# kluonj/HelFEM

Measured on AMD Instinct MI355X. Metric: scf_iteration_wall_time_fock_plus_geneig_nbf4230, lower is better.
Workload: dtype f64; 1 GPU; diatomic Z1=7 Z2=7 R=2.068 PBE, nelem=5 nnodes=15 nquad=75 lmmax=[20,20] (Nbf=4230, Nang=61, Nrad=70), XC grid 92x13, symmetry blocks [1380, 1470, 1380]: J+XC Fock build + eig_gsym_sub + density per step; parallelism=shard1, density=occupied orbitals of the core Hamiltonian

## Files before the change

### helfem_amd/csrc/hip/fock.hip

```cpp
#include "internal.h"
#include "xc_device.h"
#include "../host/dftfuncs.h"
#include "../host/fock_need.h"
#include <algorithm>
#include <cstring>

namespace hfg {

__global__ void k_gather_compact(const double *__restrict__ P, int N, int A, int R, int E, int p,
                                 const int *__restrict__ shell_off, const int *__restrict__ shell_skip,
                                 double *__restrict__ Xc, int *__restrict__ on) {
  int blk = blockIdx.x;
  int e = blk % E;
  int xy = blk / E;
  int y = xy % A, x = xy / A;
  int pp = p * p;
  int live = 0;
  for (int t = threadIdx.x; t < pp; t += blockDim.x) {
    int i = t % p, j = t / p;
    int ni = e * (p - 1) + i, nj = e * (p - 1) + j;
    double v = 0.0;
    bool ok = (ni < R) && (nj < R) && !(shell_skip[x] && ni == 0) && !(shell_skip[y] && nj == 0);
    if (ok) v = P[(size_t)(shell_off[y] + nj) * N + (shell_off[x] + ni)];
    Xc[(size_t)blk * pp + t] = v;
// ... 629 lines not shown
  if (idx >= nP * nb) return;
  double v = 0.0;
  for (int s = 0; s < nslice; s++) v += part[(size_t)s * nP * nb + idx];
  const int a = idx / nb, b = idx % nb;
  W[(size_t)(b0 + b) * nP + a] = v;
}

__global__ __launch_bounds__(256) void k_xc_density_radial(const double *__restrict__ Pc, const double *__restrict__ B,
                                                           const double *__restrict__ dB, const double *__restrict__ Lr, int A,
                                                           int E, int p, int nq, int do_grad, int do_tau, int do_lapl, int rank,
                                                           int nranks, double *__restrict__ D0, double *__restrict__ D1,
                                                           double *__restrict__ D2, double *__restrict__ D3,
                                                           const int *__restrict__ on) {
  extern __shared__ double sh[];
  const int xy = blockIdx.x, e = blockIdx.y;
  const int pp = p * p;
  if (on && !on[(size_t)xy * E + e]) {
    const size_t AA = (size_t)A * A;
    for (int q = threadIdx.x; q < nq; q += blockDim.x) {
      if ((e * nq + q) % nranks != rank) continue;
      const size_t Q = (size_t)e * nq + q;
      D0[Q * AA + xy] = 0.0;
      if (do_grad) D1[Q * AA + xy] = 0.0;
      if (do_tau) D2[Q * AA + xy] = 0.0;
      if (do_lapl) D3[Q * AA + xy] = 0.0;
    }
    return;
  }
  double *sP = sh, *sB = sh + pp, *sdB = sB + p * nq;
  const int NJ = blockDim.x / nq > 0 ? min((int)(blockDim.x / nq), p) : 1;
  double *part = sdB + p * nq;
  double *sL = part + (do_lapl ? 4 : 3) * NJ * nq;
  for (int t = threadIdx.x; t < pp; t += blockDim.x) sP[t] = Pc[((size_t)xy * E + e) * pp + t];
  for (int t = threadIdx.x; t < p * nq; t += blockDim.x) {
    int q = t / p, i = t % p;
    sB[i * nq + q] = B[((size_t)e * nq + q) * p + i];
    sdB[i * nq + q] = dB[((size_t)e * nq + q) * p + i];
    if (do_lapl) sL[i * nq + q] = Lr[((size_t)e * nq + q) * p + i];
  }
  __syncthreads();
  const size_t AA = (size_t)A * A;
  for (int q0 = 0; q0 < nq; q0 += blockDim.x / NJ) {
    const int ql = threadIdx.x % (blockDim.x / NJ), jc = threadIdx.x / (blockDim.x / NJ);
    const int q = q0 + ql;
    double d0 = 0.0, d1 = 0.0, d2 = 0.0, d3 = 0.0;
    if (q < nq && jc < NJ)
      for (int j = jc; j < p; j += NJ) {
        double s0 = 0.0, s1 = 0.0;
        for (int i = 0; i < p; i++) {
          double pv = sP[j * p + i];
          s0 += sB[i * nq + q] * pv;
          s1 += sdB[i * nq + q] * pv;
        }
        d0 += s0 * sB[j * nq + q];
        d1 += s1 * sB[j * nq + q];
        d2 += s1 * sdB[j * nq + q];
        if (do_lapl) d3 += s0 * sL[j * nq + q];
      }
    if (q < nq && jc < NJ) {
      part[(0 * NJ + jc) * nq + q] = d0;
      part[(1 * NJ + jc) * nq + q] = d1;
      part[(2 * NJ + jc) * nq + q] = d2;
      if (do_lapl) part[(3 * NJ + jc) * nq + q] = d3;
    }
    __syncthreads();
    if (jc == 0 && q < nq && (e * nq + q) % nranks == rank) {
      double a0 = 0.0, a1 = 0.0, a2 = 0.0, a3 = 0.0;
      for (int k = 0; k < NJ; k++) {
        a0 += part[(0 * NJ + k) * nq + q];
        a1 += part[(1 * NJ + k) * nq + q];
        a2 += part[(2 * NJ + k) * nq + q];
        if (do_lapl) a3 += part[(3 * NJ + k) * nq + q];
      }
      const size_t Q = (size_t)e * nq + q;
      D0[Q * AA + xy] = a0;
      if (do_grad) D1[Q * AA + xy] = a1;
      if (do_tau) D2[Q * AA + xy] = a2;
      if (do_lapl) D3[Q * AA + xy] = a3;
    }
    __syncthreads();
  }
}

__global__ void k_xc_density_theta(const double *__restrict__ D0, const double *__restrict__ D1,
                                   const double *__restrict__ D2, const double *__restrict__ D3, const double *__restrict__ Th,
                                   const double *__restrict__ dTh, const int *__restrict__ shell_l,
                                   const double *__restrict__ rad_sh, int A, int nth, int G,
                                   const int *__restrict__ grp_off, const int *__restrict__ grp_shell, int do_grad,
                                   int do_tau, int do_lapl, size_t NQ, int rank, int nranks, double *__restrict__ V, int nq,
                                   const int *__restrict__ gon) {
  extern __shared__ double sh[];
  size_t Q = blockIdx.x;
  if ((int)(Q % nranks) != rank) return;
  int ga = blockIdx.y / G, gb = blockIdx.y % G;
  if (gon && !gon[(Q / nq) * G * G + blockIdx.y]) {
    const size_t o = ((Q * G + ga) * G + gb) * nth, stride = NQ * G * G * nth;
    for (int i = threadIdx.x; i < nth; i += blockDim.x) {
      V[o + i] = 0.0;
      if (do_grad) V[stride + o + i] = V[2 * stride + o + i] = 0.0;
      if (do_tau) V[3 * stride + o + i] = V[4 * stride + o + i] = 0.0;
      if (do_lapl) V[5 * stride + o + i] = 0.0;
    }
    return;
  }
  int a0 = grp_off[ga], na = grp_off[ga + 1] - a0;
  int b0 = grp_off[gb], nb = grp_off[gb + 1] - b0;
  double *d0 = sh, *d1 = sh + na * nb, *d2 = sh + 2 * na * nb, *d3 = sh + 3 * na * nb;
  size_t AA = (size_t)A * A;
  const double ir2 = do_lapl ? 1.0 / (rad_sh[Q] * rad_sh[Q]) : 0.0;
  for (int t = threadIdx.x; t < na * nb; t += blockDim.x) {
    int ia = t / nb, ib = t % nb;
    int a = grp_shell[a0 + ia], b = grp_shell[b0 + ib];
    d0[t] = D0[Q * AA + (size_t)a * A + b];
    d1[t] = do_grad ? D1[Q * AA + (size_t)a * A + b] : 0.0;
    d2[t] = do_tau ? D2[Q * AA + (size_t)a * A + b] : 0.0;
    if (do_lapl) d3[t] = D3[Q * AA + (size_t)a * A + b] - (double)(shell_l[b] * (shell_l[b] + 1)) * ir2 * d0[t];
  }
  __syncthreads();
  for (int i = threadIdx.x; i < nth; i += blockDim.x) {
    double r = 0.0, s = 0.0, u = 0.0, k3 = 0.0, k4 = 0.0, k5 = 0.0;
    for (int ia = 0; ia < na; ia++) {
      int a = grp_shell[a0 + ia];
      double s0 = 0.0, s1 = 0.0, s2 = 0.0, s3 = 0.0, s5 = 0.0;
      for (int ib = 0; ib < nb; ib++) {
        double tb = Th[(size_t)grp_shell[b0 + ib] * nth + i];
        s0 += d0[ia * nb + ib] * tb;
        s1 += d1[ia * nb + ib] * tb;
        if (do_tau) {
          s2 += d2[ia * nb + ib] * tb;
          s3 += d0[ia * nb + ib] * dTh[(size_t)grp_shell[b0 + ib] * nth + i];
        }
        if (do_lapl) s5 += d3[ia * nb + ib] * tb;
      }
      double ta = Th[(size_t)a * nth + i];
      r += ta * s0;
      if (do_grad) {
        s += dTh[(size_t)a * nth + i] * s0;
        u += ta * s1;
      }
      if (do_tau) {
        k3 += ta * s2;
        k4 += dTh[(size_t)a * nth + i] * s3;
      }
      if (do_lapl) k5 += ta * s5;
    }
    size_t o = ((Q * G + ga) * G + gb) * nth + i;
    size_t stride = NQ * G * G * nth;
    V[o] = r;
    if (do_grad) {
      V[stride + o] = s;
      V[2 * stride + o] = u;
    }
    if (do_tau) {
      V[3 * stride + o] = k3;
      V[4 * stride + o] = k4;
    }
    if (do_lapl) V[5 * stride + o] = k5;
  }
}

template <bool EXT>
__global__ void k_xc_grid(const double *__restrict__ V, const double *__restrict__ rad_w,
                          const double *__restrict__ rad_sh, const double *__restrict__ th_s,
                          const double *__restrict__ th_w, const int *__restrict__ grp_m,
                          const double *__restrict__ cosd, const double *__restrict__ sind, int Dmax, int G, int nth,
                          int nphi, double Rh, int geom, int x_func, int c_func, int do_grad, int do_tau, int do_lapl,
                          double thr, size_t NQ, int rank, int nranks, double *__restrict__ Fo,
                          double *__restrict__ partial ) {
  extern __shared__ double sh[];
  size_t Q = blockIdx.x;
  if ((int)(Q % nranks) != rank) {
    if (threadIdx.x == 0) {
      partial[Q] = 0.0;
      partial[NQ + Q] = 0.0;
      partial[2 * NQ + Q] = 0.0;
    }
    return;
  }
  int ng = nth * nphi;
  double *p0 = sh, *p1 = sh + ng, *p2 = sh + 2 * ng, *p3 = sh + 3 * ng, *p4 = sh + 4 * ng, *p5 = sh + 5 * ng;
  double *red = sh + (do_lapl ? 6 : 5) * ng;
  double shm = rad_sh[Q], wr = rad_w[Q];
  double dphi = 2.0 * HFG_PI / nphi;
  size_t stride = NQ * G * G * nth;
  double nel = 0.0, exc_sum = 0.0, kin_sum = 0.0;
  for (int pt = threadIdx.x; pt < ng; pt += blockDim.x) {
    int i = pt / nphi, j = pt % nphi;
    double sth = th_s[i];
    double hmu, hnu, hphi, w;
    if (geom == 0) {
      double h2 = shm * shm + sth * sth;
      hmu = hnu = Rh * sqrt(h2);
      hphi = Rh * shm * sth;
      w = th_w[i] * dphi * wr * Rh * Rh * Rh * shm * h2;
    } else {
      hmu = 1.0;
      hnu = shm;
      hphi = shm * sth;
      w = th_w[i] * dphi * wr * shm * shm;
    }
    double rho = 0.0, gmu = 0.0, gnu = 0.0, gphi = 0.0, tau = 0.0, lap = 0.0;
    for (int ga = 0; ga < G; ga++)
      for (int gb = 0; gb < G; gb++) {
        int D = grp_m[ga] - grp_m[gb];
        double cd = cosd[(size_t)(D + Dmax) * nphi + j];
        size_t o = ((Q * G + ga) * G + gb) * nth + i;
        double vr = V[o];
        rho += cd * vr;
        if (do_lapl) lap += cd * V[5 * stride + o];
        if (do_tau)
          tau += 0.5 * cd * (V[3 * stride + o] / (hmu * hmu) + V[4 * stride + o] / (hnu * hnu) +
                             (double)(grp_m[ga] * grp_m[gb]) * vr / (hphi * hphi));
        if (do_grad) {
          double sd = sind[(size_t)(D + Dmax) * nphi + j];
          gnu += cd * V[stride + o];
          gmu += cd * V[2 * stride + o];
          gphi -= grp_m[ga] * sd * vr;
        }
      }
    double sigma = 0.0;
    if (do_grad) {
      gmu *= 2.0 / hmu;
      gnu *= 2.0 / hnu;
      gphi *= 2.0 / hphi;
      sigma = gmu * gmu + gnu * gnu + gphi * gphi;
    }
    double exc = 0.0, vrho = 0.0, vsig = 0.0, vtau = 0.0, vlap = 0.0;
    if (rho >= thr && rho > 0.0) {
      const bool live = 0.5 * rho >= thr;
      const double lapl = 2.0 * (2.0 * tau + lap);
      if (x_func > 0) HFG_XC_EVAL_POINT(EXT, x_func, rho, sigma, tau, lapl, live, exc, vrho, vsig, vtau, vlap);
      if (c_func > 0) HFG_XC_EVAL_POINT(EXT, c_func, rho, sigma, tau, lapl, live, exc, vrho, vsig, vtau, vlap);
      if (!isfinite(vlap)) vlap = 0.0;
    }
    nel += w * rho;
    exc_sum += w * exc * rho;
    kin_sum += w * tau;
    if (do_tau) p4[pt] = do_lapl ? w * (0.5 * vtau + 2.0 * vlap) : 0.5 * w * vtau;
    if (do_lapl) p5[pt] = w * vlap;
    p0[pt] = w * vrho;
// ... 527 lines not shown
  if (p.kind == 0) zeff = (double)p.Z;
  else if (p.kind == 1) {
    const double Hz = (p.H > 0.0) ? p.H : p.d * pow((double)(p.Z - 1), 0.4);
    zeff = 1.0 + (p.Z - 1) / (1.0 + (exp(r / p.d) - 1.0) * Hz);
  } else {
    const double alpha = 0.7280642371, beta = -0.5430794693, gamma = 0.3612163121;
    const double x = r * cbrt(128.0 * p.Z / (9.0 * HFG_PI * HFG_PI)), sx = sqrt(x);
    const double f = 1.0 + alpha * sx + beta * x * exp(-gamma * sx);
    zeff = p.Z * f * f * exp(-2.0 * alpha * sx);
  }
  const double v = -zeff / r;
  return (isfinite(v) && v != 0.0 && fabs(v) >= 2.2250738585072014e-308) ? v : 0.0;
}
__global__ void k_mp_fill(const double *__restrict__ rad_w, const double *__restrict__ rad_sh,
                          const double *__restrict__ th_c, const double *__restrict__ th_s,
                          const double *__restrict__ th_w, int G, int nth, int nphi, double Rh, int geom, DevModelPot p1,
                          DevModelPot p2, double *__restrict__ Fo) {
  const size_t Q = blockIdx.x;
  const double shm = rad_sh[Q], wr = rad_w[Q];
  const double dphi = 2.0 * HFG_PI / nphi;
  for (int t = threadIdx.x; t < G * G * nth; t += blockDim.x) {
    const int i = t % nth, gab = t / nth, ga = gab / G, gb = gab % G;
    double f = 0.0;
    if (ga == gb) {
      const double sth = th_s[i], cth = th_c[i];
      double w, v;
      if (geom == 0) {
        const double chm = sqrt(1.0 + shm * shm);
        w = th_w[i] * dphi * wr * Rh * Rh * Rh * shm * (shm * shm + sth * sth);
        v = mp_potential(p1, Rh * (chm + cth)) + mp_potential(p2, Rh * (chm - cth));
      } else {
        w = th_w[i] * dphi * wr * shm * shm;
        v = mp_potential(p1, shm);
      }
      f = 0.5 * nphi * w * v;
    }
    Fo[((Q * G + ga) * G + gb) * nth + i] = f;
  }
}

static int round_up64(int n) { return ((n + 63) / 64) * 64; }
static size_t xc_fock_radial_lds(int p, int nq, int do_lapl = 0) {
  const size_t shb = (size_t)(4 * nq + (do_lapl ? 6 : 4) * nq * p) * sizeof(double);
  if (shb > 150 * 1024) throw std::runtime_error("radial quadrature too large for the XC Fock kernel's LDS tables");
  if (shb > 64 * 1024)
    HFG_HIP_CHECK(hipFuncSetAttribute((const void *)k_xc_fock_radial, hipFuncAttributeMaxDynamicSharedMemorySize, (int)shb));
  return shb;
}
static size_t xc_fock_theta_lds(int nth, int maxgrp, int do_lapl) {
  size_t shb = (size_t)((do_lapl ? 6 : 5) * nth + 4 * nth * maxgrp) * sizeof(double);
  if (shb > 160 * 1024) throw std::runtime_error("angular grid too large for the XC Fock kernel's LDS tables");
  if (shb > 64 * 1024)
    HFG_HIP_CHECK(hipFuncSetAttribute((const void *)k_xc_fock_theta, hipFuncAttributeMaxDynamicSharedMemorySize, (int)shb));
  return shb;
}
static void launch_xc_fock_theta(hfg_ctx *ctx, size_t NQ, int G, int nth, int maxgrp, const double *Fo, const double *Th, const double *dTh,
                                 int A, const int *grp_off, const int *grp_shell, int do_grad, int do_tau, int rank, int nranks,
                                 double *GA, double *GB, double *GC, int do_lapl = 0, double *GL = nullptr, const int *gneed = nullptr) {
  const int nf = do_lapl ? 6 : 5;
  const size_t need = (size_t)(nf * nth + 4 * nth * maxgrp) * sizeof(double);
  if (need <= tuning().xc_lds_limit) {
    hipLaunchKernelGGL(k_xc_fock_theta, dim3((unsigned)NQ, G * G), dim3(256), xc_fock_theta_lds(nth, maxgrp, do_lapl), ctx->stream, Fo, Th, dTh, A,
                       nth, G, grp_off, grp_shell, do_grad, do_tau, do_lapl, NQ, rank, nranks, GA, GB, GC, GL, gneed);
    return;
  }
  if (maxgrp * maxgrp > XC_FT_MAXPP * 256) throw std::runtime_error("angular basis too large for the XC Fock kernels (more than 64 shells of one m)");
  int nthc = (int)(tuning().xc_lds_limit / sizeof(double) / (nf + 4 * maxgrp));
  if (nthc < 4) throw std::runtime_error("angular basis too large for the XC Fock kernels' LDS tables");
  nthc = std::min(nthc, nth);
  const size_t shb = (size_t)(nf * nthc + 4 * nthc * maxgrp) * sizeof(double);
  if (do_lapl) {
    if (shb > 64 * 1024)
      HFG_HIP_CHECK(hipFuncSetAttribute((const void *)k_xc_fock_theta_chunked<true>, hipFuncAttributeMaxDynamicSharedMemorySize, (int)shb));
    hipLaunchKernelGGL(k_xc_fock_theta_chunked<true>, dim3((unsigned)NQ, G * G), dim3(256), shb, ctx->stream, Fo, Th, dTh, A, nth, G, grp_off,
                       grp_shell, do_grad, do_tau, NQ, rank, nranks, GA, GB, GC, GL, nthc, gneed);
    return;
  }
  if (shb > 64 * 1024)
    HFG_HIP_CHECK(hipFuncSetAttribute((const void *)k_xc_fock_theta_chunked<false>, hipFuncAttributeMaxDynamicSharedMemorySize, (int)shb));
  hipLaunchKernelGGL(k_xc_fock_theta_chunked<false>, dim3((unsigned)NQ, G * G), dim3(256), shb, ctx->stream, Fo, Th, dTh, A, nth, G, grp_off,
                     grp_shell, do_grad, do_tau, NQ, rank, nranks, GA, GB, GC, (double *)nullptr, nthc, gneed);
}

static size_t xc_density_radial_lds(int p, int nq, int do_lapl = 0) {
  const int NJ = (256 / nq > 0) ? std::min(256 / nq, p) : 1;
  size_t shb = (size_t)(p * p + 2 * p * nq + 3 * NJ * nq + (do_lapl ? NJ * nq + p * nq : 0)) * sizeof(double);
  if (shb > 150 * 1024) throw std::runtime_error("radial quadrature too large for the XC density kernel's LDS tables");
  if (shb > 64 * 1024)
    HFG_HIP_CHECK(hipFuncSetAttribute((const void *)k_xc_density_radial, hipFuncAttributeMaxDynamicSharedMemorySize, (int)shb));
  return shb;
}

struct FockAux : Workspace {
  DevBuf<int> pure_shell, pure_n, lmpos;
  DevBuf<double> Pc, Jc, Pc2, Jc2, Pc3, Paux, Y, Jaux, D0, D1, D2, D3, V, Fo, GA, GB, GC, GL, partial, scal;
  DevBuf<int> on, gon, chan;
};

struct FockSkip {
  const int *on = nullptr, *gon = nullptr;
  int *chan = nullptr;
  const int *need = nullptr, *gneed = nullptr;
};

static void aux_setup(hfg_ctx *ctx, const hfg_dev_tables *t, FockAux *a) {
  std::vector<int> ps(t->N), pn(t->N);
  {
    size_t k = 0;
    for (int s = 0; s < t->A; s++)
      for (int n = (t->h_shell_skip[s] ? 1 : 0); n < t->R; n++, k++) {
        ps[k] = s;
        pn[k] = n;
      }
  }
  a->pure_shell.upload(ps, ctx->stream);
  a->pure_n.upload(pn, ctx->stream);
  std::vector<int> lmpos(2 * t->Nlm, -1);
  for (int i = 0; i < t->NLM; i++) {
    int M = t->h_LM_M[i];
    int ilm = t->h_LM_ilm[i];
    if (M >= 0) lmpos[2 * ilm] = i;
    if (M < 0) lmpos[2 * ilm + 1] = i;
  }
  a->lmpos.upload(lmpos, ctx->stream);
  HFG_HIP_CHECK(hipStreamSynchronize(ctx->stream));
}
static FockAux &aux_for(hfg_ctx *ctx, hfg_basis *basis) {
  hfg_dev_tables *t = basis->dev;
  return t->work.get<FockAux>(WS_FOCK, [&](FockAux &a) { aux_setup(ctx, t, &a); });
}

static hfg_dev_tables *tables_of(hfg_ctx *ctx, hfg_basis *basis) {
  if (!basis->dev || !basis->dev->have_tei) throw std::logic_error("Primitive teis have not been computed!\n");
  if (basis->dev_device != ctx->device) throw std::logic_error("basis tables live on a different device\n");
  return basis->dev;
}

static void gather_compact(hfg_ctx *ctx, hfg_basis *basis, const double *dP, double *dPc) {
  hfg_dev_tables *t = basis->dev;
  hipLaunchKernelGGL(k_gather_compact, dim3(t->A * t->A * t->E), dim3(256), 0, ctx->stream, dP, t->N, t->A, t->R, t->E,
                     t->p, t->shell_off.p, t->shell_skip.p, dPc, (int *)nullptr);
}

static void skip_flags_behind_on(hfg_ctx *ctx, hfg_dev_tables *t, FockAux &a, bool with_need, FockSkip &sk) {
  sk.on = a.on.p;
  sk.chan = a.chan.p;
  if (t->have_xc) {
    a.gon.resize((size_t)t->E * t->G * t->G);
    hipLaunchKernelGGL(k_skip_groups, dim3(t->E, t->G * t->G), dim3(256), 0, ctx->stream, a.on.p, t->A, t->E, t->G, t->grp_off.p,
                       t->grp_shell.p, a.gon.p);
    sk.gon = a.gon.p;
  }
  if (with_need && ctx->fock_need_tables == t && ctx->fock_need_A == t->A) {
    sk.need = ctx->fock_need.p;
    if (t->have_xc && ctx->fock_need_G == t->G) sk.gneed = ctx->fock_gneed.p;
  }
}

static FockSkip gather_compact_flagged(hfg_ctx *ctx, hfg_basis *basis, const double *dP, double *dPc, bool with_need) {
  hfg_dev_tables *t = basis->dev;
  FockSkip sk;
  if (!helfem::tuning_live().fock_skip) {
    gather_compact(ctx, basis, dP, dPc);
    return sk;
  }
  FockAux &a = aux_for(ctx, basis);
// ... 149 lines not shown
    w.Pc.resize(nb * nc);
    w.Jc.resize(nb * nc);
    for (int b = 0; b < nb; b++) gather_compact(ctx, basis, dP + (size_t)(b0 + b) * N2, w.Pc.p + b * nc);
    coulomb_batch_compact(ctx, basis, nb, w.Pc.p, w.Jc.p);
    for (int b = 0; b < nb; b++) scatter_dense(ctx, basis, w.Jc.p + b * nc, dJ + (size_t)(b0 + b) * N2);
  }
  HFG_HIP_CHECK(hipGetLastError());
}

void coulomb_energy_matrix_dev(hfg_ctx *ctx, hfg_basis *basis, int64_t nP, const double *dP, double *dW) {
  if (nP <= 0) return;
  hfg_dev_tables *t = tables_of(ctx, basis);
  CoulombBatchAux &w = batch_aux_for(basis);
  const size_t nc = (size_t)t->A * t->A * t->E * t->p * t->p, N2 = (size_t)t->N * t->N;
  const int64_t chunk = coulomb_batch_chunk(t);
  const unsigned nslice = (unsigned)((nc + CB_SLICE - 1) / CB_SLICE);
  ProfScope ps(ctx, "coulomb_batch");
  w.Pc.resize(nP * nc);
  w.Jc.resize(std::min(chunk, nP) * nc);
  w.part.resize((size_t)nslice * nP * std::min(chunk, nP));
  for (int64_t b = 0; b < nP; b++) gather_compact(ctx, basis, dP + (size_t)b * N2, w.Pc.p + b * nc);
  for (int64_t b0 = 0; b0 < nP; b0 += chunk) {
    const int nb = (int)std::min(chunk, nP - b0);
    coulomb_batch_compact(ctx, basis, nb, w.Pc.p + b0 * nc, w.Jc.p);
    hipLaunchKernelGGL(k_coulomb_energy_part, dim3(nslice, (unsigned)((nP + CB_WT - 1) / CB_WT), (nb + CB_WT - 1) / CB_WT), dim3(256), 0,
                       ctx->stream, w.Pc.p, (int)nP, w.Jc.p, nb, nc, w.part.p);
    hipLaunchKernelGGL(k_coulomb_energy_sum, dim3((unsigned)((nP * nb + 255) / 256)), dim3(256), 0, ctx->stream, w.part.p, (int)nslice,
                       (int)nP, nb, (int)b0, dW);
  }
  HFG_HIP_CHECK(hipGetLastError());
}

struct XCPlan {
  int do_grad, do_tau, do_lapl;
  bool ext;
  double thr;
  int maxgrp;
  size_t NQ, AA, nv;
};
static XCPlan xc_plan(const hfg_dev_tables *t, int x_func, int c_func, double thr) {
  if (!t->have_xc) throw std::runtime_error("XC grid tables were not uploaded (hfg_basis_upload with ldft,mdft > 0)\n");
  auto either = [&](bool (*is)(int)) { return (x_func > 0 && is(x_func)) || (c_func > 0 && is(c_func)); };
  if ((x_func > 0 && !xc::is_supported(x_func)) || (c_func > 0 && !xc::is_supported(c_func)))
    throw std::runtime_error("Functional not found!");
  XCPlan pl;
  pl.do_grad = either(xc::is_gga);
  pl.do_lapl = either(xc::is_mgga_lapl);
  if (pl.do_lapl && t->geom != 1) throw std::logic_error("Laplacian not implemented!\n");
  pl.do_tau = either(xc::is_mgga) || pl.do_lapl;
  pl.ext = either(xc::is_ext);
  pl.thr = pl.do_tau ? std::max(thr, 1e-40) : thr;
  pl.maxgrp = 0;
  for (int g = 0; g < t->G; g++) pl.maxgrp = std::max(pl.maxgrp, t->h_grp_off[g + 1] - t->h_grp_off[g]);
  pl.NQ = (size_t)t->E * t->nq;
  pl.AA = (size_t)t->A * t->A;
  pl.nv = pl.NQ * t->G * t->G * t->ntheta;
  return pl;
}

static void xc_buffers(FockAux &a, const XCPlan &pl, int planes) {
  a.D0.resize(pl.NQ * pl.AA);
  a.D1.resize(pl.NQ * pl.AA);
  a.GA.resize(pl.NQ * pl.AA);
  a.GB.resize(pl.NQ * pl.AA);
  if (pl.do_tau) {
    a.D2.resize(pl.NQ * pl.AA);
    a.GC.resize(pl.NQ * pl.AA);
  }
  if (pl.do_lapl) {
    a.D3.resize(pl.NQ * pl.AA);
    a.GL.resize(pl.NQ * pl.AA);
  }
  a.V.resize(planes * pl.nv);
  a.Fo.resize(planes * pl.nv);
  a.partial.resize(3 * pl.NQ);
}

static void xc_density_stage(hfg_ctx *ctx, const hfg_dev_tables *t, FockAux &a, const XCPlan &pl, const double *dPc, double *dV,
                             const FockSkip &sk = FockSkip()) {
  const int A = t->A, E = t->E, p = t->p, nq = t->nq, G = t->G, nth = t->ntheta;
  hipLaunchKernelGGL(k_xc_density_radial, dim3(A * A, E), dim3(256), xc_density_radial_lds(p, nq, pl.do_lapl), ctx->stream, dPc,
                     t->rad_B.p, t->rad_dB.p, (const double *)t->rad_L.p, A, E, p, nq, pl.do_grad, pl.do_tau, pl.do_lapl,
                     ctx->shard_rank, ctx->shard_n, a.D0.p, a.D1.p, a.D2.p, a.D3.p, sk.on);
  hipLaunchKernelGGL(k_xc_density_theta, dim3((unsigned)pl.NQ, G * G), dim3(std::min(256, round_up64(nth))),
                     (pl.do_lapl ? 4 : 3) * pl.maxgrp * pl.maxgrp * sizeof(double), ctx->stream, a.D0.p, a.D1.p, (const double *)a.D2.p,
                     (const double *)a.D3.p, t->Th.p, t->dTh.p, t->shell_l.p, t->rad_sh.p, A, nth, G, t->grp_off.p, t->grp_shell.p,
                     pl.do_grad, pl.do_tau, pl.do_lapl, pl.NQ, ctx->shard_rank, ctx->shard_n, dV, nq, sk.gon);
}

static void xc_fock_stage(hfg_ctx *ctx, const hfg_dev_tables *t, FockAux &a, const XCPlan &pl, double *dFo, double *dHc,
                          const FockSkip &sk = FockSkip()) {
  const int A = t->A, E = t->E, p = t->p, nq = t->nq;
  launch_xc_fock_theta(ctx, pl.NQ, t->G, t->ntheta, pl.maxgrp, dFo, t->Th.p, t->dTh.p, A, t->grp_off.p, t->grp_shell.p, pl.do_grad,
                       pl.do_tau, ctx->shard_rank, ctx->shard_n, a.GA.p, a.GB.p, a.GC.p, pl.do_lapl, a.GL.p, sk.gneed);
  hipLaunchKernelGGL(k_xc_fock_radial, dim3(A * A, E), dim3(std::min(256, round_up64(p * p))), xc_fock_radial_lds(p, nq, pl.do_lapl),
                     ctx->stream, a.GA.p, a.GB.p, (const double *)a.GC.p, (const double *)a.GL.p, t->rad_B.p, t->rad_dB.p,
                     (const double *)t->rad_L.p, t->shell_l.p, t->rad_sh.p, A, E, p, nq, pl.do_grad, pl.do_tau, pl.do_lapl, ctx->shard_rank,
                     ctx->shard_n, dHc, sk.need);
}

template <typename K, typename... Tail>
static void launch_xc_grid(hfg_ctx *ctx, const hfg_dev_tables *t, FockAux &a, const XCPlan &pl, K k_ext, K k_plain, size_t shb,
                           int x_func, int c_func, Tail... tail) {
  K k = pl.ext ? k_ext : k_plain;
  if (shb > 64 * 1024) HFG_HIP_CHECK(hipFuncSetAttribute((const void *)k, hipFuncAttributeMaxDynamicSharedMemorySize, (int)shb));
  hipLaunchKernelGGL(k, dim3((unsigned)pl.NQ), dim3(256), shb, ctx->stream, a.V.p, t->rad_w.p, t->rad_sh.p, t->th_s.p, t->th_w.p,
                     t->grp_m.p, t->cosd.p, t->sind.p, t->Dmax, t->G, t->ntheta, t->nphi, t->Rhalf, t->geom, x_func, c_func, pl.do_grad,
                     pl.do_tau, pl.do_lapl, pl.thr, pl.NQ, ctx->shard_rank, ctx->shard_n, a.Fo.p, a.partial.p, tail...);
}

static void xc_compact(hfg_ctx *ctx, hfg_basis *basis, int x_func, int c_func, const double *dPc, double *dHc, double *dScal,
                       double thr, const FockSkip &sk = FockSkip()) {
  hfg_dev_tables *t = tables_of(ctx, basis);
  const XCPlan pl = xc_plan(t, x_func, c_func, thr);
  FockAux &a = aux_for(ctx, basis);
  const int npl = pl.do_lapl ? 6 : 5;
  xc_buffers(a, pl, npl);
  xc_density_stage(ctx, t, a, pl, dPc, a.V.p, sk);
  size_t shb = (size_t)(npl * t->ntheta * t->nphi + 3 * 4) * sizeof(double);
  if (pl.do_lapl && shb > 150 * 1024) throw std::runtime_error("XC angular grid too large for the grid kernel's LDS planes");
  launch_xc_grid(ctx, t, a, pl, k_xc_grid<true>, k_xc_grid<false>, shb, x_func, c_func);
  xc_fock_stage(ctx, t, a, pl, a.Fo.p, dHc, sk);
  hipLaunchKernelGGL(k_xc_sum_partials, dim3(1), dim3(64), 0, ctx->stream, a.partial.p, pl.NQ, dScal);
  HFG_HIP_CHECK(hipGetLastError());
}

static void fill_xcpar(xc::XCPar &par, int id, const double *pars, int n) {
  const helfem::XCFunc *f = helfem::find_xc_func(id);
  const char *name = f ? f->pars : "";
  for (int i = 0; i < n; i++) {
    const size_t len = strcspn(name, ",");
    double *field = nullptr;
#define FIELD(m) \
  if (len == strlen(#m) && !strncmp(name, #m, len)) field = &par.m;
    FIELD(x_alpha) FIELD(x_kappa) FIELD(x_mu) FIELD(c_beta) FIELD(c_gamma) FIELD(c_BB) FIELD(x_omega)
#undef FIELD
    if (!field) throw std::logic_error("xc_funcs.h names an XCPar field that does not exist\n");
    if (field == &par.x_omega && !(pars[i] > 0.0)) throw std::runtime_error("The range-separation constant omega must be positive.\n");
    *field = pars[i];
    name += len + (name[len] == ',');
  }
}

void set_xc_params(hfg_ctx *ctx, int x_func, const double *x_pars, int nx, int c_func, const double *c_pars, int nc) {
  xc::XCPar par = HFG_XCPAR_DEFAULTS;
  if (nx > 0 && !x_pars) throw std::runtime_error("Exchange functional parameters missing.\n");
  if (nc > 0 && !c_pars) throw std::runtime_error("Correlation functional parameters missing.\n");
  helfem::check_xc_params(x_func, nx, c_func, nc);
  fill_xcpar(par, x_func, x_pars, nx);
  fill_xcpar(par, c_func, c_pars, nc);
  static thread_local xc::XCPar staged[8];
  static thread_local int slot = 0;
  staged[slot] = par;
  HFG_HIP_CHECK(hipMemcpyToSymbolAsync(HIP_SYMBOL(xc::c_xcpar), &staged[slot], sizeof(par), 0, hipMemcpyHostToDevice, ctx->stream));
  slot = (slot + 1) % 8;
}

void xc_eval_host(int id, int nspin, size_t np, const double *rho, const double *sigma, const double *lapl, const double *tau,
                  double *exc, double *vrho, double *vsigma, double *vlapl, double *vtau, double thr) {
  if (id <= 0 || !xc::is_supported(id)) throw std::runtime_error("Functional not found!");
  if (nspin != 1 && nspin != 2) throw std::logic_error("hfg_xc_eval: nspin must be 1 or 2\n");
  if (!rho) throw std::logic_error("hfg_xc_eval: rho is required\n");
  if (xc::is_mgga(id) || xc::is_mgga_lapl(id)) thr = std::max(thr, 1e-40);
  auto in = [](const double *a, size_t i) { return a ? a[i] : 0.0; };
  auto out = [](double *a, size_t i, double v) {
    if (a) a[i] = v;
  };
  for (size_t i = 0; i < np; i++) {
    if (nspin == 1) {
      const double r = rho[i], s = in(sigma, i), l = in(lapl, i), t = in(tau, i);
// ... 310 lines not shown
```

Baseline: 7.696 ms.

## Register-block XC density theta kernel with chunked shell sums and wave slicing

Rewrites the angular density contraction kernel so each thread accumulates up to 16 a-shells at once in registers. Theta values for b-shells are prefetched in groups of four, and shell indices are cached in LDS. When nth is small (one tile, 13 theta points here), the a-shell range is split across the four waves and their partial sums are combined through LDS. The kernel is templated on tau/laplacian and always launches 256 threads, aiming to cut repeated global loads and the idle waves of a 64-thread block. The cost is extra register pressure, a second barrier, and more template instantiations.

```diff
diff --git a/helfem_amd/csrc/hip/fock.hip b/helfem_amd/csrc/hip/fock.hip
--- a/helfem_amd/csrc/hip/fock.hip
+++ b/helfem_amd/csrc/hip/fock.hip
@@ -735,80 +735,186 @@
   }
 }
 
-__global__ void k_xc_density_theta(const double *__restrict__ D0, const double *__restrict__ D1,
-                                   const double *__restrict__ D2, const double *__restrict__ D3, const double *__restrict__ Th,
-                                   const double *__restrict__ dTh, const int *__restrict__ shell_l,
-                                   const double *__restrict__ rad_sh, int A, int nth, int G,
-                                   const int *__restrict__ grp_off, const int *__restrict__ grp_shell, int do_grad,
-                                   int do_tau, int do_lapl, size_t NQ, int rank, int nranks, double *__restrict__ V, int nq,
-                                   const int *__restrict__ gon) {
+constexpr int XC_DT_CH = 16;
+constexpr int XC_DT_NB = 4;
+__host__ __device__ inline int xc_dt_tiles(int nth) { return (nth + 63) / 64; }
+__host__ __device__ inline int xc_dt_slices(int nth) { return xc_dt_tiles(nth) >= 4 ? 1 : 4 / xc_dt_tiles(nth); }
+
+template <int NC, bool TAU, bool LAPL>
+__device__ __forceinline__ void xc_dt_chunk(const double *__restrict__ Th, const double *__restrict__ dTh, const double *d0,
+                                            const double *d1, const double *d2, const double *d3, const int *sa, const int *sb,
+                                            int c0, int nc, int nb, int nth, int ic, int do_grad, double (&v)[6]) {
+  double s0[NC], s1[NC], s2[TAU ? NC : 1], s3[TAU ? NC : 1], s5[LAPL ? NC : 1];
+#pragma unroll
+  for (int j = 0; j < NC; j++) {
+    s0[j] = s1[j] = 0.0;
+    if (TAU) s2[TAU ? j : 0] = s3[TAU ? j : 0] = 0.0;
+    if (LAPL) s5[LAPL ? j : 0] = 0.0;
+  }
+  double tb[XC_DT_NB], db[TAU ? XC_DT_NB : 1], tn[XC_DT_NB], dn[TAU ? XC_DT_NB : 1];
+#pragma unroll
+  for (int u = 0; u < XC_DT_NB; u++) {
+    const size_t ob = (size_t)sb[min(u, nb - 1)] * nth + ic;
+    tb[u] = Th[ob];
+    if (TAU) db[TAU ? u : 0] = dTh[ob];
+  }
+  for (int ib = 0; ib < nb; ib += XC_DT_NB) {
+#pragma unroll
+    for (int u = 0; u < XC_DT_NB; u++) {
+      const size_t ob = (size_t)sb[min(ib + XC_DT_NB + u, nb - 1)] * nth + ic;
+      tn[u] = Th[ob];
+      if (TAU) dn[TAU ? u : 0] = dTh[ob];
+    }
+#pragma unroll
+    for (int u = 0; u < XC_DT_NB; u++) {
+      if (ib + u < nb) {
+#pragma unroll
+        for (int j = 0; j < NC; j++) {
+          const int t = (c0 + min(j, nc - 1)) * nb + ib + u;
+          s0[j] += d0[t] * tb[u];
+          s1[j] += d1[t] * tb[u];
+          if (TAU) {
+            s2[TAU ? j : 0] += d2[t] * tb[u];
+            s3[TAU ? j : 0] += d0[t] * db[TAU ? u : 0];
+          }
+          if (LAPL) s5[LAPL ? j : 0] += d3[t] * tb[u];
+        }
+      }
+    }
+#pragma unroll
+    for (int u = 0; u < XC_DT_NB; u++) {
+      tb[u] = tn[u];
+      if (TAU) db[TAU ? u : 0] = dn[TAU ? u : 0];
+    }
+  }
+#pragma unroll
+  for (int j0 = 0; j0 < NC; j0 += 4) {
+    double ta[4], da[4];
+#pragma unroll
+    for (int j = 0; j < 4; j++) {
+      const size_t oa = (size_t)sa[c0 + min(j0 + j, nc - 1)] * nth + ic;
+      ta[j] = Th[oa];
+      da[j] = dTh[oa];
+    }
+#pragma unroll
+    for (int j = 0; j < 4; j++) {
+      if (j0 + j < nc) {
+        v[0] += ta[j] * s0[j0 + j];
+        if (do_grad) {
+          v[1] += da[j] * s0[j0 + j];
+          v[2] += ta[j] * s1[j0 + j];
+        }
+        if (TAU) {
+          v[3] += ta[j] * s2[TAU ? j0 + j : 0];
+          v[4] += da[j] * s3[TAU ? j0 + j : 0];
+        }
+        if (LAPL) v[5] += ta[j] * s5[LAPL ? j0 + j : 0];
+      }
+    }
+  }
+}
+
+template <bool TAU, bool LAPL>
+__device__ __forceinline__ void xc_dt_point(const double *__restrict__ Th, const double *__restrict__ dTh, const double *d0,
+                                            const double *d1, const double *d2, const double *d3, const int *sa, const int *sb,
+                                            int lo, int hi, int nb, int nth, int ic, int do_grad, double (&v)[6]) {
+  for (int c0 = lo; c0 < hi; c0 += XC_DT_CH) {
+    const int nc = min(XC_DT_CH, hi - c0);
+    if (nc > 12)
+      xc_dt_chunk<16, TAU, LAPL>(Th, dTh, d0, d1, d2, d3, sa, sb, c0, nc, nb, nth, ic, do_grad, v);
+    else if (nc > 8)
+      xc_dt_chunk<12, TAU, LAPL>(Th, dTh, d0, d1, d2, d3, sa, sb, c0, nc, nb, nth, ic, do_grad, v);
+    else if (nc > 4)
+      xc_dt_chunk<8, TAU, LAPL>(Th, dTh, d0, d1, d2, d3, sa, sb, c0, nc, nb, nth, ic, do_grad, v);
+    else
+      xc_dt_chunk<4, TAU, LAPL>(Th, dTh, d0, d1, d2, d3, sa, sb, c0, nc, nb, nth, ic, do_grad, v);
+  }
+}
+
+template <bool TAU, bool LAPL>
+__device__ __forceinline__ void xc_dt_store(double *__restrict__ V, size_t o, size_t stride, int do_grad, const double (&v)[6]) {
+  V[o] = v[0];
+  if (do_grad) {
+    V[stride + o] = v[1];
+    V[2 * stride + o] = v[2];
+  }
+  if (TAU) {
+    V[3 * stride + o] = v[3];
+    V[4 * stride + o] = v[4];
+  }
+  if (LAPL) V[5 * stride + o] = v[5];
+}
+
+template <bool TAU, bool LAPL>
+__global__ __launch_bounds__(256) __attribute__((amdgpu_waves_per_eu(TAU ? 2 : 4))) void k_xc_density_theta(const double *__restrict__ D0, const double *__restrict__ D1,
+                                                          const double *__restrict__ D2, const double *__restrict__ D3,
+                                                          const double *__restrict__ Th, const double *__restrict__ dTh,
+                                                          const int *__restrict__ shell_l, const double *__restrict__ rad_sh, int A,
+                                                          int nth, int G, const int *__restrict__ grp_off,
+                                                          const int *__restrict__ grp_shell, int do_grad, size_t NQ, int rank,
+                                                          int nranks, double *__restrict__ V, int nq, const int *__restrict__ gon) {
   extern __shared__ double sh[];
   size_t Q = blockIdx.x;
   if ((int)(Q % nranks) != rank) return;
   int ga = blockIdx.y / G, gb = blockIdx.y % G;
+  const size_t stride = NQ * G * G * nth, o = ((Q * G + ga) * G + gb) * nth;
   if (gon && !gon[(Q / nq) * G * G + blockIdx.y]) {
-    const size_t o = ((Q * G + ga) * G + gb) * nth, stride = NQ * G * G * nth;
     for (int i = threadIdx.x; i < nth; i += blockDim.x) {
       V[o + i] = 0.0;
       if (do_grad) V[stride + o + i] = V[2 * stride + o + i] = 0.0;
-      if (do_tau) V[3 * stride + o + i] = V[4 * stride + o + i] = 0.0;
-      if (do_lapl) V[5 * stride + o + i] = 0.0;
+      if (TAU) V[3 * stride + o + i] = V[4 * stride + o + i] = 0.0;
+      if (LAPL) V[5 * stride + o + i] = 0.0;
     }
     return;
   }
+  constexpr int ND = 2 + (TAU ? 1 : 0) + (LAPL ? 1 : 0), NV = 3 + (TAU ? 2 : 0) + (LAPL ? 1 : 0);
+  const int ntile = xc_dt_tiles(nth), NS = xc_dt_slices(nth), np = 64 * ntile;
   int a0 = grp_off[ga], na = grp_off[ga + 1] - a0;
   int b0 = grp_off[gb], nb = grp_off[gb + 1] - b0;
-  double *d0 = sh, *d1 = sh + na * nb, *d2 = sh + 2 * na * nb, *d3 = sh + 3 * na * nb;
+  const int nn = na * nb;
+  double *d0 = sh, *d1 = sh + nn, *d2 = sh + 2 * nn, *d3 = sh + (ND - 1) * nn;
+  double *red = sh + ND * nn;
+  int *sa = (int *)(red + (NS - 1) * NV * np), *sb = sa + na;
   size_t AA = (size_t)A * A;
-  const double ir2 = do_lapl ? 1.0 / (rad_sh[Q] * rad_sh[Q]) : 0.0;
-  for (int t = threadIdx.x; t < na * nb; t += blockDim.x) {
+  const double ir2 = LAPL ? 1.0 / (rad_sh[Q] * rad_sh[Q]) : 0.0;
+  for (int t = threadIdx.x; t < na; t += blockDim.x) sa[t] = grp_shell[a0 + t];
+  for (int t = threadIdx.x; t < nb; t += blockDim.x) sb[t] = grp_shell[b0 + t];
+  for (int t = threadIdx.x; t < nn; t += blockDim.x) {
     int ia = t / nb, ib = t % nb;
     int a = grp_shell[a0 + ia], b = grp_shell[b0 + ib];
     d0[t] = D0[Q * AA + (size_t)a * A + b];
     d1[t] = do_grad ? D1[Q * AA + (size_t)a * A + b] : 0.0;
-    d2[t] = do_tau ? D2[Q * AA + (size_t)a * A + b] : 0.0;
-    if (do_lapl) d3[t] = D3[Q * AA + (size_t)a * A + b] - (double)(shell_l[b] * (shell_l[b] + 1)) * ir2 * d0[t];
+    if (TAU) d2[t] = D2[Q * AA + (size_t)a * A + b];
+    if (LAPL) d3[t] = D3[Q * AA + (size_t)a * A + b] - (double)(shell_l[b] * (shell_l[b] + 1)) * ir2 * d0[t];
   }
   __syncthreads();
-  for (int i = threadIdx.x; i < nth; i += blockDim.x) {
-    double r = 0.0, s = 0.0, u = 0.0, k3 = 0.0, k4 = 0.0, k5 = 0.0;
-    for (int ia = 0; ia < na; ia++) {
-      int a = grp_shell[a0 + ia];
-      double s0 = 0.0, s1 = 0.0, s2 = 0.0, s3 = 0.0, s5 = 0.0;
-      for (int ib = 0; ib < nb; ib++) {
-        double tb = Th[(size_t)grp_shell[b0 + ib] * nth + i];
-        s0 += d0[ia * nb + ib] * tb;
-        s1 += d1[ia * nb + ib] * tb;
-        if (do_tau) {
-          s2 += d2[ia * nb + ib] * tb;
-          s3 += d0[ia * nb + ib] * dTh[(size_t)grp_shell[b0 + ib] * nth + i];
-        }
-        if (do_lapl) s5 += d3[ia * nb + ib] * tb;
-      }
-      double ta = Th[(size_t)a * nth + i];
-      r += ta * s0;
-      if (do_grad) {
-        s += dTh[(size_t)a * nth + i] * s0;
-        u += ta * s1;
-      }
-      if (do_tau) {
-        k3 += ta * s2;
-        k4 += dTh[(size_t)a * nth + i] * s3;
-      }
-      if (do_lapl) k5 += ta * s5;
-    }
-    size_t o = ((Q * G + ga) * G + gb) * nth + i;
-    size_t stride = NQ * G * G * nth;
-    V[o] = r;
-    if (do_grad) {
-      V[stride + o] = s;
-      V[2 * stride + o] = u;
-    }
-    if (do_tau) {
-      V[3 * stride + o] = k3;
-      V[4 * stride + o] = k4;
-    }
-    if (do_lapl) V[5 * stride + o] = k5;
+  const int wave = __builtin_amdgcn_readfirstlane(threadIdx.x >> 6), lane = threadIdx.x & 63;
+  if (NS == 1) {
+    for (int tile = wave; tile < ntile; tile += 4) {
+      const int i = tile * 64 + lane;
+      double v[6] = {0.0, 0.0, 0.0, 0.0, 0.0, 0.0};
+      xc_dt_point<TAU, LAPL>(Th, dTh, d0, d1, d2, d3, sa, sb, 0, na, nb, nth, min(i, nth - 1), do_grad, v);
+      if (i < nth) xc_dt_store<TAU, LAPL>(V, o + i, stride, do_grad, v);
+    }
+    return;
+  }
+  const int tile = wave % ntile, sl = wave / ntile, nsl = (na + NS - 1) / NS;
+  const int i = tile * 64 + lane;
+  double v[6] = {0.0, 0.0, 0.0, 0.0, 0.0, 0.0};
+  xc_dt_point<TAU, LAPL>(Th, dTh, d0, d1, d2, d3, sa, sb, min(na, sl * nsl), min(na, (sl + 1) * nsl), nb, nth, min(i, nth - 1),
+                         do_grad, v);
+  if (sl > 0) {
+#pragma unroll
+    for (int k = 0; k < 6; k++)
+      if (k < 3 || (TAU && k < 5) || (LAPL && k == 5)) red[((sl - 1) * NV + (k == 5 ? NV - 1 : k)) * np + i] = v[k];
+  }
+  __syncthreads();
+  if (sl == 0 && i < nth) {
+    for (int s = 1; s < NS; s++)
+#pragma unroll
+      for (int k = 0; k < 6; k++)
+        if (k < 3 || (TAU && k < 5) || (LAPL && k == 5)) v[k] += red[((s - 1) * NV + (k == 5 ? NV - 1 : k)) * np + i];
+    xc_dt_store<TAU, LAPL>(V, o + i, stride, do_grad, v);
   }
 }
 
@@ -1502,6 +1608,14 @@
                      grp_shell, do_grad, do_tau, NQ, rank, nranks, GA, GB, GC, (double *)nullptr, nthc, gneed);
 }
 
+static size_t xc_density_theta_lds(const void *k, int nth, int maxgrp, int do_tau, int do_lapl) {
+  const size_t nd = 2 + (do_tau ? 1 : 0) + (do_lapl ? 1 : 0), nv = 3 + (do_tau ? 2 : 0) + (do_lapl ? 1 : 0);
+  const size_t shb = (nd * maxgrp * maxgrp + (xc_dt_slices(nth) - 1) * nv * 64 * xc_dt_tiles(nth)) * sizeof(double) + 2 * maxgrp * sizeof(int);
+  if (shb > 160 * 1024) throw std::runtime_error("angular basis too large for the XC density kernel's LDS tables");
+  if (shb > 64 * 1024) HFG_HIP_CHECK(hipFuncSetAttribute(k, hipFuncAttributeMaxDynamicSharedMemorySize, (int)shb));
+  return shb;
+}
+
 static size_t xc_density_radial_lds(int p, int nq, int do_lapl = 0) {
   const int NJ = (256 / nq > 0) ? std::min(256 / nq, p) : 1;
   size_t shb = (size_t)(p * p + 2 * p * nq + 3 * NJ * nq + (do_lapl ? NJ * nq + p * nq : 0)) * sizeof(double);
@@ -1817,10 +1931,11 @@
   hipLaunchKernelGGL(k_xc_density_radial, dim3(A * A, E), dim3(256), xc_density_radial_lds(p, nq, pl.do_lapl), ctx->stream, dPc,
                      t->rad_B.p, t->rad_dB.p, (const double *)t->rad_L.p, A, E, p, nq, pl.do_grad, pl.do_tau, pl.do_lapl,
                      ctx->shard_rank, ctx->shard_n, a.D0.p, a.D1.p, a.D2.p, a.D3.p, sk.on);
-  hipLaunchKernelGGL(k_xc_density_theta, dim3((unsigned)pl.NQ, G * G), dim3(std::min(256, round_up64(nth))),
-                     (pl.do_lapl ? 4 : 3) * pl.maxgrp * pl.maxgrp * sizeof(double), ctx->stream, a.D0.p, a.D1.p, (const double *)a.D2.p,
-                     (const double *)a.D3.p, t->Th.p, t->dTh.p, t->shell_l.p, t->rad_sh.p, A, nth, G, t->grp_off.p, t->grp_shell.p,
-                     pl.do_grad, pl.do_tau, pl.do_lapl, pl.NQ, ctx->shard_rank, ctx->shard_n, dV, nq, sk.gon);
+  auto k = pl.do_lapl ? k_xc_density_theta<true, true> : pl.do_tau ? k_xc_density_theta<true, false> : k_xc_density_theta<false, false>;
+  hipLaunchKernelGGL(k, dim3((unsigned)pl.NQ, G * G), dim3(256), xc_density_theta_lds((const void *)k, nth, pl.maxgrp, pl.do_tau, pl.do_lapl),
+                     ctx->stream, a.D0.p, a.D1.p, (const double *)a.D2.p, (const double *)a.D3.p, t->Th.p, t->dTh.p, t->shell_l.p,
+                     t->rad_sh.p, A, nth, G, t->grp_off.p, t->grp_shell.p, pl.do_grad, pl.NQ, ctx->shard_rank, ctx->shard_n, dV, nq,
+                     sk.gon);
 }
 
 static void xc_fock_stage(hfg_ctx *ctx, const hfg_dev_tables *t, FockAux &a, const XCPlan &pl, double *dFo, double *dHc,
```

Result: no change. 7.633 ms (median of 6 runs) (-0.8%).
